# Yubo-Shankui/Bind-Your-Avatar-Implementation

Measured on AMD Instinct MI355X. Metric: denoise-steps/sec, higher is better.
Workload: dtype bf16; 1 GPU; BASELINE.json configs[1]: full transformer.forward, 49x480x720 (13x30x45 latent tokens + 226 text), 2 characters (2 ID + 2 audio), batch 1, random-init 8.6B-param architecture; layers=42, batch=1, launch=eager, parallelism=single GPU

## Files before the change

### bind_your_avatar_implementation_amd/_hip.py

```python
import ctypes
import os

from .build import LIB_PATH as _BUILT_LIB

LIB_PATH = os.environ.get("BYA_HIP_LIB") or _BUILT_LIB

_c = ctypes
_vp, _i32, _i64, _f32 = _c.c_void_p, _c.c_int32, _c.c_int64, _c.c_float


class GemmDesc(_c.Structure):
    _fields_ = [("M", _i32), ("N", _i32), ("K", _i32), ("batch", _i32),
                ("lda", _i32), ("ldw", _i32), ("ldc", _i32), ("ldres", _i32),
                ("a_batch_stride", _i64), ("c_batch_stride", _i64), ("res_batch_stride", _i64),
                ("gate_batch_stride", _i64), ("gate_split", _i32), ("act", _i32),
                ("n_split", _i32), ("c_split_stride", _i64), ("bias_rowscale", _vp), ("alpha", _f32)]


class GemmPlan(_c.Structure):
    _fields_ = [("path", _i32), ("m0", _i32), ("tail", _i32), ("split_k", _i32), ("row_chunks", _i32)]


class QkNormDesc(_c.Structure):
    _fields_ = [("qw", _vp), ("qb", _vp), ("kw", _vp), ("kb", _vp), ("cos", _vp), ("sin", _vp),
# ... 96 lines not shown
    "bya_masks_to_routing_logits": [_vp, _vp, _i32, _i32, _i32, _i32, _i32, _i32, _i32, _vp],
    "bya_vae_patches": [_vp, _vp, _vp] + [_i32] * 14 + [_vp],
    "bya_vae_groupnorm_stats": [_vp, _vp, _vp, _i64, _i32, _i32, _vp],
    "bya_vae_norm_act": [_vp, _vp, _vp, _vp, _vp, _vp, _vp, _i64, _i32, _i32, _i32, _f32, _i32, _i32, _i32, _i32, _i32, _i32,
                         _i32, _i64, _i32, _vp],
    "bya_vae_conv3d": [_vp, _vp, _vp, _vp, _vp, _i32, _i32, _i32, _i32, _i32, _i32, _i64, _i64, _i64, _vp],
    "bya_vae_upsample_pad": [_vp, _vp, _i32, _i32, _i32, _i32, _i32, _vp],
    "bya_allgather_kv": [_vp, _vp, _vp, _vp, _i64, _i64, _vp, _vp],
    "bya_alltoall_router": [_vp, _vp, _vp, _vp, _i32, _vp, _vp],
    "bya_p2p_push": [_vp, _i32, _i64, _vp, _i32, _i32, _vp, _vp],
    "bya_p2p_wait": [_vp, _i32, _vp, _i64, _vp],
    "bya_p2p_exchange": [_vp, _i32, _i64, _vp, _i32, _i32, _vp, _vp, _i64, _vp],
    "bya_p2p_poison": [_vp, _i32, _vp, _i64, _vp],
    "bya_p2p_alloc": [_i64, _i32, _c.POINTER(_vp)],
    "bya_p2p_free": [_vp],
    "bya_p2p_ipc_export": [_vp, _vp],
    "bya_p2p_ipc_import": [_vp, _c.POINTER(_vp)],
    "bya_p2p_ipc_release": [_vp],
    "bya_cfg_scheduler_step": [_vp, _i32, _i64, _vp, _vp, _vp, _vp, _vp, _i64, _c.POINTER(SchedCoef), _vp],
}

OPTIONS = {"gemm_splitk": 0, "gemm_splitk_min": 1, "gemm_tile": 2, "gemm_variant": 3, "attn_streamk": 4, "fp8_kernel": 5,
           "p2p_groups": 6, "reference_forms": 7}
REFERENCE_FORMS = {"rowgemm_chunked": 1, "kv_mix_generic": 2, "ln_generic": 4, "router_scores_wave": 8, "attn_narrow_store": 16}
ENV_OPTIONS = {
    "BYA_GEMM_SPLITK": ("gemm_splitk", int),
    "BYA_GEMM_SPLITK_MIN": ("gemm_splitk_min", int),
    "BYA_GEMM_TILE": ("gemm_tile", int),
    "BYA_GEMM_VARIANT": ("gemm_variant", lambda v: {"w8": 1, "no128": 2}.get(v, 0)),
    "BYA_ATTN_STREAMK": ("attn_streamk", int),
    "BYA_FP8_KERNEL": ("fp8_kernel", lambda v: 1 if v.startswith("1") else 0),
    "BYA_P2P_GROUPS": ("p2p_groups", int),
}

GEMM_PATHS = {0: "t128x64", 1: "t128x128", 2: "t256x128", 3: "t256x256", 4: "p256", 5: "p128", 6: "p128s", 7: "w8_256"}

ATTN_VARIANTS = {0: "d64_running_max", 1: "d64_prescaled_running_max", 2: "d64_static_bound", 3: "d128_running_max",
                 4: "d64_static_bound_w4", 5: "d64_device_bound_w4"}
KV_MIX_FORMS = {0: "mix32", 1: "one_tile"}
TINY_INSTANCES = {0: "tiny8<2>", 1: "tiny8<3>", 2: "tiny8<13>", 3: "tiny8<25>", 4: "generic<2>", 5: "generic<4>",
                  6: "generic<16>", 7: "generic<32>"}

ERRORS = {-1: "BYA_ERR_SHAPE", -2: "BYA_ERR_ALIGN", -3: "BYA_ERR_LAUNCH", -4: "BYA_ERR_UNSUPPORTED"}

_lib = None


# ... 47 lines not shown
```

### bind_your_avatar_implementation_amd/csrc/misc.hip

```cpp
#include "bya_common.h"
#include "../../include/bya.h"
#include "options.h"
#include "routing_weights.h"

namespace {

template <int MAXM>
__global__ __launch_bounds__(256) void linear_small_m_kernel(const bf16_t* __restrict__ x, const bf16_t* __restrict__ W,
                                                             const bf16_t* __restrict__ bias, bf16_t* __restrict__ out,
                                                             int M, int N, int K, int silu_in, int act_out) {
    const int lane = threadIdx.x & 63;
    const long long n = (long long)blockIdx.x * 4 + (threadIdx.x >> 6);
    if (n >= N) return;
    float acc[MAXM];
#pragma unroll
    for (int m = 0; m < MAXM; ++m) acc[m] = 0.f;
    const bf16_t* wrow = W + n * K;
    for (int k0 = lane * 8; k0 < K; k0 += 512) {
        float wv[8];
        unpack8(*reinterpret_cast<const u32x4*>(wrow + k0), wv);
#pragma unroll
        for (int m = 0; m < MAXM; ++m) {
            if (m < M) {
                float xv[8];
// ... 273 lines not shown
        v += plane(lt.i1) * lt.w1;
        if (v > 0.5f) label = id;
    }
    for (int id = 0; id < n_id; ++id) out[tok * n_id + id] = (id == label) ? (bf16_t)0x3F80 : (bf16_t)0;
}

}

extern "C" int bya_abi_version(void) { return 2; }

std::atomic<int32_t> g_bya_options[BYA_OPT_COUNT] = {
    {0},
    {0},
    {-1},
    {0},
    {1},
    {0},
    {0},
    {0},
};

extern "C" int bya_set_option(int32_t key, int32_t value) {
    static const int32_t lo[BYA_OPT_COUNT] = {0, 0, -1, 0, 0, 0, 0, 0};
    static const int32_t hi[BYA_OPT_COUNT] = {2, 1 << 20, 6, 2, 1, 1, 1024, 31};
    if (key < 0 || key >= BYA_OPT_COUNT || value < lo[key] || value > hi[key]) return BYA_ERR_SHAPE;
    if (key == BYA_OPT_P2P_GROUPS && value != 0 && value < 16) return BYA_ERR_SHAPE;
    g_bya_options[key].store(value, std::memory_order_relaxed);
    return BYA_OK;
}

extern "C" int bya_get_option(int32_t key, int32_t* value) {
    if (key < 0 || key >= BYA_OPT_COUNT || !value) return BYA_ERR_SHAPE;
    *value = g_bya_options[key].load(std::memory_order_relaxed);
    return BYA_OK;
}

extern "C" int bya_linear_small_m(const void* x, const void* W, const void* bias, void* out, int32_t M, int32_t N,
                                  int32_t K, int32_t silu_in, int32_t act_out, hipStream_t stream) {
    if (!x || !W || !out || M <= 0 || M > 8 || N <= 0 || K <= 0) return BYA_ERR_SHAPE;
    if (K % 8) return BYA_ERR_SHAPE;
    if (((uintptr_t)x | (uintptr_t)W) & 15) return BYA_ERR_ALIGN;
    if (act_out != BYA_ACT_NONE && act_out != BYA_ACT_SILU) return BYA_ERR_UNSUPPORTED;
    dim3 grid((unsigned)((N + 3) / 4));
    if (M <= 2)
        BYA_LAUNCH((linear_small_m_kernel<2>), grid, dim3(256), 0, stream, (const bf16_t*)x, (const bf16_t*)W,
                           (const bf16_t*)bias, (bf16_t*)out, M, N, K, silu_in, act_out);
    else
// ... 116 lines not shown
```

### bind_your_avatar_implementation_amd/csrc/rowgemm.hip

```cpp
#include "rowgemm_common.h"
#include "../../include/bya.h"
#include "options.h"

#ifndef BYA_ROWGEMM_ABLATE
#define BYA_ROWGEMM_ABLATE 0
#endif

namespace {

using namespace rowk;

struct RowGemmArgs {
    const bf16_t* X; const bf16_t* W; const float* colsum; const float* cvec; const bf16_t* res; bf16_t* C;
    int M, N, ldx, ldc, ldres;
    float eps;
};

constexpr int HB = 2;
constexpr int NW = CH / (4 * HB);
constexpr int SR = CH / NW;
constexpr int RB = 16 * HB * NW;
constexpr int WG_PER_CU = 1;
constexpr int AHEAD = 1;

template <bool LN, bool RES, int ACT>
__global__ __launch_bounds__(64 * NW, 2) void rowgemm512_kernel(RowGemmArgs p) {
    extern __shared__ __attribute__((aligned(16))) char smem[];
    const int tid = threadIdx.x, lane = tid & 63;
    const int wave = __builtin_amdgcn_readfirstlane(tid >> 6);

    const int nrb = (p.M + RB - 1) / RB, ncc = p.N / CH;
    const long long total = (long long)nrb * ncc;
    const int rid = (gridDim.x & 7) == 0 ? (int)((blockIdx.x & 7) * (gridDim.x >> 3) + (blockIdx.x >> 3)) : (int)blockIdx.x;
    const int q0 = (int)(total * rid / gridDim.x), q1 = (int)(total * (rid + 1) / gridDim.x);
    if (q0 >= q1) return;

    float* s_lds = reinterpret_cast<float*>(smem);
    float* c_lds = s_lds + p.N;
    char* ring = smem + p.N * 8;
    for (int i = tid; i < p.N; i += 64 * NW) {
        s_lds[i] = LN ? p.colsum[i] : 0.0f;
        c_lds[i] = p.cvec[i];
    }
    __syncthreads();

    const __amdgpu_buffer_rsrc_t rsX = __builtin_amdgcn_make_buffer_rsrc(
        (void*)p.X, 0, (int)(((long long)(p.M - 1) * p.ldx + RK) * 2), 0x00020000);
    const __amdgpu_buffer_rsrc_t rsW = __builtin_amdgcn_make_buffer_rsrc((void*)p.W, 0, p.N * RK * 2, 0x00020000);
    const __amdgpu_buffer_rsrc_t rsC = __builtin_amdgcn_make_buffer_rsrc(
        (void*)p.C, 0, (int)(((long long)(p.M - 1) * p.ldc + p.N) * 2), 0x00020000);
    const __amdgpu_buffer_rsrc_t rsR = __builtin_amdgcn_make_buffer_rsrc(
        (void*)(RES ? p.res : p.C), 0, (int)(((long long)(p.M - 1) * (RES ? p.ldres : p.ldc) + p.N) * 2), 0x00020000);
// ... 44 lines not shown
                for (int h = 0; h < HB; ++h) {
                    f32x4 sm = {0.f, 0.f, 0.f, 0.f}, gr = {0.f, 0.f, 0.f, 0.f};
#pragma unroll
                    for (int ks = 0; ks < 16; ++ks) {
                        sm = __builtin_amdgcn_mfma_f32_16x16x32_bf16(ones, xf[h][ks], sm, 0, 0, 0);
                        gr = __builtin_amdgcn_mfma_f32_16x16x32_bf16(xf[h][ks], xf[h][ks], gr, 0, 0, 0);
                    }
                    const int e = to & 3;
                    const float d = e == 0 ? gr[0] : e == 1 ? gr[1] : e == 2 ? gr[2] : gr[3];
                    const float sq = __shfl(d, (int)(to + 16 * (to >> 2)));
                    const float mu = sm[0] * (1.0f / RK);
                    const float var = fmaxf(sq * (1.0f / RK) - mu * mu, 0.0f);
                    mean[h] = mu;
                    rstd[h] = rsqrtf(var + p.eps);
                }
            }
        }
        asm volatile("s_waitcnt vmcnt(0)" ::: "memory");
#pragma unroll
        for (int h = 0; h < HB; ++h)
#pragma unroll
            for (int ks = 0; ks < 16; ++ks) asm volatile("" : "+v"(xf[h][ks]));

        for (; q < qe; ++q, ++it) {
            const int cc = q - rb * ncc, stg = it & 1;
            const uint32_t ln = lane_now(), to = ln & 15u, go = ln >> 4;
            asm volatile("s_waitcnt vmcnt(%0)" ::"i"(NJ * HB / 2) : "memory");
            __builtin_amdgcn_s_barrier();
            u32x4 rv[HB][NJ / 2];
            if (RES) {
#pragma unroll
                for (int h = 0; h < HB; ++h)
#pragma unroll
                    for (int u = 0; u < NJ / 2; ++u)
                        rv[h][u] = __builtin_bit_cast(u32x4, __builtin_amdgcn_raw_buffer_load_b128(
                            rsR, ((uint32_t)(r0 + h * 16) + to) * (uint32_t)(p.ldres * 2) +
                                     ((uint32_t)(cc * CH) + lane_col(go, u)) * 2, 0, 0));
            }
            if (q + 1 < q1) stage_chunk(q + 1, stg ^ 1);

            uint32_t wa[4];
#pragma unroll
            for (int m = 0; m < 4; ++m)
                wa[m] = ring_base + stg * STAGE_BYTES + to * 1024 + (((go ^ (to & 3)) | ((m ^ (to >> 2)) << 2)) << 4);
            f32x4 acc[HB][NJ];
#pragma unroll
            for (int h = 0; h < HB; ++h)
#pragma unroll
                for (int j = 0; j < NJ; ++j) acc[h][j] = f32x4{0.f, 0.f, 0.f, 0.f};
            bf16x8 wf[AHEAD + 1][NJ];
#pragma unroll
            for (int a = 0; a < AHEAD; ++a) read_kstep(wf[a], wa, a);
#pragma unroll
            for (int ks = 0; ks < 16; ++ks) {
                const int cur = ks % (AHEAD + 1);
                if (ks + AHEAD < 16) {
                    read_kstep(wf[(ks + AHEAD) % (AHEAD + 1)], wa, ks + AHEAD);
                    lgkm_wait<AHEAD * NJ>(wf[cur]);
                } else if (ks + 1 < 16 && AHEAD == 2) {
                    lgkm_wait<NJ>(wf[cur]);
                } else {
                    lgkm_wait<0>(wf[cur]);
                }
#pragma unroll
                for (int j = 0; j < NJ; ++j)
#pragma unroll
                    for (int h = 0; h < HB; ++h)
                        acc[h][j] = __builtin_amdgcn_mfma_f32_16x16x32_bf16(wf[cur][j], xf[h][ks], acc[h][j], 0, 0, 0);
            }

#pragma unroll
            for (int u = 0; u < NJ / 2; ++u) {
                f32x4 s0, s1, c0, c1;
                const uint32_t a = smem_base + ((uint32_t)(cc * CH) + lane_col(go, u)) * 4, ac = a + (uint32_t)p.N * 4;
                lds_read_f<0>(s0, a);
                lds_read_f<16>(s1, a);
                lds_read_f<0>(c0, ac);
                lds_read_f<16>(c1, ac);
                asm volatile("s_waitcnt lgkmcnt(0)" : "+v"(s0), "+v"(s1), "+v"(c0), "+v"(c1));
#pragma unroll
                for (int h = 0; h < HB; ++h) {
                    float v[8];
#pragma unroll
                    for (int e = 0; e < 8; ++e) {
                        const float a0 = acc[h][2 * u + (e >> 2)][e & 3];
                        const float sv = (e >> 2) ? s1[e & 3] : s0[e & 3];
                        const float cv = (e >> 2) ? c1[e & 3] : c0[e & 3];
                        float o = LN ? fmaf(rstd[h], fmaf(-mean[h], sv, a0), cv) : a0 + cv;
                        if (ACT == BYA_ACT_GELU_ERF) o = gelu_erf_f(o);
                        if (RES) o += (e & 1) ? bfhi(rv[h][u][e >> 1]) : bflo(rv[h][u][e >> 1]);
                        v[e] = o;
                    }
                    u32x4 ov;
#pragma unroll
                    for (int w2 = 0; w2 < 4; ++w2) ov[w2] = pack2bf(v[2 * w2], v[2 * w2 + 1]);
#if BYA_ROWGEMM_ABLATE & 2
                    if (ov[0] == 0x12345678u && ov[3] == 0x9abcdef0u)
#endif
                    __builtin_amdgcn_raw_buffer_store_b128(ov, rsC, ((uint32_t)(r0 + h * 16) + to) * (uint32_t)(p.ldc * 2) +
                                                                        ((uint32_t)(cc * CH) + lane_col(go, u)) * 2, 0, 0);
                }
            }
        }
    }
}

template <bool LN, bool RES, int ACT>
int launch_rowgemm(const RowGemmArgs& a, hipStream_t s) {
    const long long total = (long long)((a.M + RB - 1) / RB) * (a.N / CH);
    const int blocks = (int)(total < 256 * WG_PER_CU ? total : 256 * WG_PER_CU);
    const size_t lds = (size_t)a.N * 8 + 2 * STAGE_BYTES;
    static std::atomic<unsigned long long> attr_done{0};
    if (bya_allow_big_lds(reinterpret_cast<const void*>(rowgemm512_kernel<LN, RES, ACT>), 160 * 1024, attr_done) != BYA_OK)
        return BYA_ERR_LAUNCH;
    BYA_LAUNCH((rowgemm512_kernel<LN, RES, ACT>), dim3(blocks), dim3(64 * NW), lds, s, a);
    return hipGetLastError() == hipSuccess ? BYA_OK : BYA_ERR_LAUNCH;
}


template <bool LN, bool RES, int ACT>
__global__ __launch_bounds__(64 * NW, 2) void rowgemm512q_kernel(RowGemmArgs p) {
    static_assert(!LN, "the W-stationary form has no LayerNorm-folding instance");
    extern __shared__ __attribute__((aligned(16))) char smem[];
    const int tid = threadIdx.x, lane = tid & 63;
    const int wave = __builtin_amdgcn_readfirstlane(tid >> 6);
    const int xcd = blockIdx.x & 7, idx = blockIdx.x >> 3, per_xcd = gridDim.x >> 5;
    const int quarter = idx & 3, rgrp = xcd * per_xcd + (idx >> 2), ngroups = gridDim.x >> 2;
    const int col_base = quarter * 128;

    float* s_lds = reinterpret_cast<float*>(smem);
    float* c_lds = s_lds + 128;
    char* ring = smem + 1024;
    if (tid < 128) {
        s_lds[tid] = LN ? p.colsum[col_base + tid] : 0.0f;
        c_lds[tid] = p.cvec[col_base + tid];
    }
    const __amdgpu_buffer_rsrc_t rsX = __builtin_amdgcn_make_buffer_rsrc(
        (void*)p.X, 0, (int)(((long long)(p.M - 1) * p.ldx + RK) * 2), 0x00020000);
    const __amdgpu_buffer_rsrc_t rsW = __builtin_amdgcn_make_buffer_rsrc((void*)p.W, 0, p.N * RK * 2, 0x00020000);
// ... 185 lines not shown
#pragma unroll
        for (int j = 0; j < NJ; ++j) acc[h][j] = f32x4{0.f, 0.f, 0.f, 0.f};
    bf16x8 wf[AHEAD + 1][NJ];
#pragma unroll
    for (int a = 0; a < AHEAD; ++a) read_kstep(wf[a], wa, a);
#pragma unroll
    for (int ks = 0; ks < 16; ++ks) {
        const int cur = ks % (AHEAD + 1);
        if (ks + AHEAD < 16) {
            read_kstep(wf[(ks + AHEAD) % (AHEAD + 1)], wa, ks + AHEAD);
            lgkm_wait<AHEAD * NJ>(wf[cur]);
        } else {
            lgkm_wait<0>(wf[cur]);
        }
#pragma unroll
        for (int j = 0; j < NJ; ++j)
#pragma unroll
            for (int h = 0; h < HB; ++h)
                acc[h][j] = SWAP ? __builtin_amdgcn_mfma_f32_16x16x32_bf16(xf[h][ks], wf[cur][j], acc[h][j], 0, 0, 0)
                                 : __builtin_amdgcn_mfma_f32_16x16x32_bf16(wf[cur][j], xf[h][ks], acc[h][j], 0, 0, 0);
    }
}

template <bool WIDE>
__global__ __launch_bounds__(64 * NW, 2) void rowattn512_kernel(RowAttnArgs p) {
    extern __shared__ __attribute__((aligned(16))) char smem[];
    const int tid = threadIdx.x, lane = tid & 63;
    const int wave = __builtin_amdgcn_readfirstlane(tid >> 6);

    const long long tiles = WIDE ? 2 * p.n_groups : (p.n_groups + p.G - 1) / p.G;
    const int nrb = (int)((tiles + NW * HB - 1) / (NW * HB));
    const int total = nrb * RA_HEADS;
    const int rid = (gridDim.x & 7) == 0 ? (int)((blockIdx.x & 7) * (gridDim.x >> 3) + (blockIdx.x >> 3)) : (int)blockIdx.x;
    const int u0 = (int)((long long)total * rid / gridDim.x), u1 = (int)((long long)total * (rid + 1) / gridDim.x);
    if (u0 >= u1) return;

    float* s_lds = reinterpret_cast<float*>(smem);
    float* c_lds = s_lds + RA_N;
    float* st_lds = c_lds + RA_N + wave * (HB * 32);
    char* ring = smem + RA_CONST_BYTES;
    for (int i = tid; i < RA_N; i += 64 * NW) {
        s_lds[i] = p.colsum[i];
        c_lds[i] = p.cvec[i];
    }
    __syncthreads();

    const __amdgpu_buffer_rsrc_t rsX = __builtin_amdgcn_make_buffer_rsrc(
        (void*)p.X, 0, (int)(((long long)(p.M - 1) * p.ldx + RK) * 2), 0x00020000);
    const __amdgpu_buffer_rsrc_t rsW = __builtin_amdgcn_make_buffer_rsrc((void*)p.W, 0, RA_N * RK * 2, 0x00020000);
    const __amdgpu_buffer_rsrc_t rsO = __builtin_amdgcn_make_buffer_rsrc(
        (void*)p.O, 0, (int)(((long long)(p.M - 1) * p.ldo + RK) * 2), 0x00020000);
// ... 61 lines not shown
                for (int ks = 0; ks < 16; ++ks) {
                    sm = __builtin_amdgcn_mfma_f32_16x16x32_bf16(ones, xf[h][ks], sm, 0, 0, 0);
                    gr = __builtin_amdgcn_mfma_f32_16x16x32_bf16(xf[h][ks], xf[h][ks], gr, 0, 0, 0);
                }
                const int e = to & 3;
                const float d = e == 0 ? gr[0] : e == 1 ? gr[1] : e == 2 ? gr[2] : gr[3];
                const float sq = __shfl(d, (int)(to + 16 * (to >> 2)));
                const float mu = sm[0] * (1.0f / RK);
                const float var = fmaxf(sq * (1.0f / RK) - mu * mu, 0.0f);
                mean[h] = mu;
                rstd[h] = rsqrtf(var + p.eps);
                if (go == 0) {
                    st_lds[h * 32 + to] = mean[h];
                    st_lds[h * 32 + 16 + to] = rstd[h];
                }
            }
        }
        asm volatile("s_waitcnt vmcnt(0) lgkmcnt(0)" ::: "memory");
#pragma unroll
        for (int h = 0; h < HB; ++h)
#pragma unroll
            for (int ks = 0; ks < 16; ++ks) asm volatile("" : "+v"(xf[h][ks]));

        for (; u < ue; ++u) {
            const int head = u & (RA_HEADS - 1);
            u32x4 qf[HB][2], kf[HB][2];
            u32x2 pf[HB][WIDE ? HB : 1];
            float invl[HB];
#pragma unroll
            for (int part = 0; part < 2; ++part) {
                const uint32_t ln = lane_now(), to = ln & 15u, go = ln >> 4;
                if (part == 0) asm volatile("s_waitcnt vmcnt(%0)" ::"i"(2 * HB) : "memory");
                else asm volatile("s_waitcnt vmcnt(0)" ::: "memory");
                __builtin_amdgcn_s_barrier();
                if (3 * u + part + 1 < q_end) stage_chunk(3 * u + part + 1, stg ^ 1);
                uint32_t wa[4];
#pragma unroll
                for (int m = 0; m < 4; ++m)
                    wa[m] = ring_base + stg * STAGE_BYTES + to * 1024 + (((go ^ (to & 3)) | ((m ^ (to >> 2)) << 2)) << 4);
                f32x4 acc[HB][NJ];
                rowattn_chunk<false>(acc, xf, wa);
                const uint32_t sc_base = smem_base + (uint32_t)(part * 512 + head * 64 + LPC * go) * 4;
#pragma unroll
                for (int kb = 0; kb < 2; ++kb) {
                    f32x4 s0, s1, c0, c1;
                    const uint32_t a = sc_base + (uint32_t)(8 * kb) * 4, ac = a + (uint32_t)RA_N * 4;
                    lds_read_f<0>(s0, a);
                    lds_read_f<16>(s1, a);
                    lds_read_f<0>(c0, ac);
                    lds_read_f<16>(c1, ac);
                    asm volatile("s_waitcnt lgkmcnt(0)" : "+v"(s0), "+v"(s1), "+v"(c0), "+v"(c1));
#pragma unroll
                    for (int h = 0; h < HB; ++h) {
                        float v[8];
#pragma unroll
                        for (int e = 0; e < 8; ++e) {
                            const float a0 = acc[h][2 * kb + (e >> 2)][e & 3];
                            const float sv = (e >> 2) ? s1[e & 3] : s0[e & 3];
                            const float cv = (e >> 2) ? c1[e & 3] : c0[e & 3];
                            v[e] = fmaf(rstd[h], fmaf(-mean[h], sv, a0), cv);
                        }
                        u32x4 w;
#pragma unroll
                        for (int w2 = 0; w2 < 4; ++w2) w[w2] = pack2bf(v[2 * w2], v[2 * w2 + 1]);
                        if (part == 0) qf[h][kb] = w; else kf[h][kb] = w;
                    }
                }
                stg ^= 1;
            }
            constexpr int NKT = WIDE ? HB : 1;
#pragma unroll
            for (int h = 0; h < HB; ++h) {
                float sv[NKT][4];
                float mx = -INFINITY;
#pragma unroll
                for (int hk = 0; hk < NKT; ++hk) {
                    const int kt = WIDE ? hk : h;
                    f32x4 st = {0.f, 0.f, 0.f, 0.f};
#pragma unroll
                    for (int kb = 0; kb < 2; ++kb)
                        st = __builtin_amdgcn_mfma_f32_16x16x32_bf16(__builtin_bit_cast(bf16x8, kf[kt][kb]),
                                                                     __builtin_bit_cast(bf16x8, qf[h][kb]), st, 0, 0, 0);
#pragma unroll
                    for (int e = 0; e < 4; ++e) {
                        sv[hk][e] = (kmask >> (4 * hk + e)) & 1u ? st[e] : -INFINITY;
                        mx = fmaxf(mx, sv[hk][e]);
                    }
                }
                mx = fmaxf(mx, __shfl_xor(mx, 16));
                mx = fmaxf(mx, __shfl_xor(mx, 32));
                float l = 0.f;
#pragma unroll
                for (int hk = 0; hk < NKT; ++hk) {
                    float pe[4];
#pragma unroll
                    for (int e = 0; e < 4; ++e) {
                        pe[e] = __builtin_amdgcn_exp2f((sv[hk][e] - mx) * p.scale_log2);
                        l += pe[e];
                    }
                    pf[h][hk][0] = pack2bf(pe[0], pe[1]);
                    pf[h][hk][1] = pack2bf(pe[2], pe[3]);
                }
                l += __shfl_xor(l, 16);
                l += __shfl_xor(l, 32);
                invl[h] = __builtin_amdgcn_rcpf(l);
            }
            {
                const uint32_t ln = lane_now(), to = ln & 15u, go = ln >> 4;
                asm volatile("s_waitcnt vmcnt(0)" ::: "memory");
                __builtin_amdgcn_s_barrier();
                if (3 * u + 3 < q_end) stage_chunk(3 * u + 3, stg ^ 1);
                uint32_t wa[4];
#pragma unroll
                for (int m = 0; m < 4; ++m)
                    wa[m] = ring_base + stg * STAGE_BYTES + to * 1024 + (((go ^ (to & 3)) | ((m ^ (to >> 2)) << 2)) << 4);
                f32x4 acc[HB][NJ];
                rowattn_chunk<true>(acc, xf, wa);
                const uint32_t col = (uint32_t)(1024 + head * 64) + LPC * (to >> 2) + (to & 3);
                float sj[NJ], cj[NJ];
#pragma unroll
                for (int j = 0; j < NJ; ++j) {
                    sj[j] = s_lds[col + 4 * j];
                    cj[j] = c_lds[col + 4 * j];
                }
                auto make_vt = [&](int h, u32x2 (&vt)[NJ]) {
                    f32x4 m4, r4;
                    lds_read_f<0>(m4, st_base + (uint32_t)(h * 32 + 4 * go) * 4);
                    lds_read_f<64>(r4, st_base + (uint32_t)(h * 32 + 4 * go) * 4);
                    asm volatile("s_waitcnt lgkmcnt(0)" : "+v"(m4), "+v"(r4));
#pragma unroll
                    for (int j = 0; j < NJ; ++j) {
                        float vv[4];
#pragma unroll
                        for (int e = 0; e < 4; ++e) vv[e] = fmaf(r4[e], fmaf(-m4[e], sj[j], acc[h][j][e]), cj[j]);
                        vt[j][0] = pack2bf(vv[0], vv[1]);
                        vt[j][1] = pack2bf(vv[2], vv[3]);
                    }
                };
                u32x2 vt[WIDE ? HB : 1][NJ];
                if constexpr (WIDE) {
#pragma unroll
                    for (int h = 0; h < HB; ++h) make_vt(h, vt[h]);
                }
#pragma unroll
                for (int h = 0; h < HB; ++h) {
                    if constexpr (!WIDE) make_vt(h, vt[0]);
                    float ov[16];
#pragma unroll
                    for (int j = 0; j < NJ; ++j) {
                        f32x4 o = {0.f, 0.f, 0.f, 0.f};
#pragma unroll
                        for (int hk = 0; hk < NKT; ++hk)
                            o = __builtin_amdgcn_mfma_f32_16x16x16bf16_1k(__builtin_bit_cast(s16x4, vt[WIDE ? hk : 0][j]),
                                                                          __builtin_bit_cast(s16x4, pf[h][hk]), o, 0, 0, 0);
#pragma unroll
                        for (int e = 0; e < 4; ++e) ov[4 * j + e] = o[e] * invl[h];
                    }
                    const uint32_t off = rowi[h] * (uint32_t)(p.ldo * 2) + ((uint32_t)(head * 64) + LPC * go) * 2;
                    __builtin_amdgcn_raw_buffer_store_b128(pack8(ov), rsO, off, 0, 0);
                    __builtin_amdgcn_raw_buffer_store_b128(pack8(ov + 8), rsO, off + 16, 0, 0);
                }
                stg ^= 1;
            }
        }
    }
}

}

extern "C" int bya_rowgemm512(const void* X, const void* W, const float* colsum, const float* cvec, const void* res,
                              void* C, int32_t M, int32_t N, int32_t ldx, int32_t ldc, int32_t ldres, int32_t ln,
                              float eps, int32_t act, int32_t nsplit, hipStream_t stream) {
    (void)nsplit;
    if (!X || !W || !cvec || !C || M <= 0 || N <= 0) return BYA_ERR_SHAPE;
    if (ln && !colsum) return BYA_ERR_SHAPE;
    if (N % CH != 0 || N > 4096) return BYA_ERR_SHAPE;
    if (ldx < RK || ldc < N || (res && ldres < N) || ldx % 8 || ldc % 8 || (res && ldres % 8)) return BYA_ERR_ALIGN;
    if (((uintptr_t)X | (uintptr_t)W | (uintptr_t)C | (uintptr_t)res) & 15) return BYA_ERR_ALIGN;
    if ((long long)M * ldx * 2 >= (1LL << 31) || (long long)M * ldc * 2 >= (1LL << 31)) return BYA_ERR_SHAPE;
    if (act != BYA_ACT_NONE && act != BYA_ACT_GELU_ERF) return BYA_ERR_UNSUPPORTED;
    RowGemmArgs a;
    a.X = (const bf16_t*)X; a.W = (const bf16_t*)W; a.colsum = colsum; a.cvec = cvec; a.res = (const bf16_t*)res;
    a.C = (bf16_t*)C; a.M = M; a.N = N; a.ldx = ldx; a.ldc = ldc; a.ldres = res ? ldres : ldc;
    a.eps = eps;
    const bool gelu = act == BYA_ACT_GELU_ERF;
    if (N == 512 && !ln && M >= 2048 && M <= 65536 && !bya_ref_form(BYA_REF_ROWGEMM_CHUNKED)) {
        if (res) return gelu ? launch_rowgemm_q<false, true, BYA_ACT_GELU_ERF>(a, stream) : launch_rowgemm_q<false, true, BYA_ACT_NONE>(a, stream);
// ... 13 lines not shown

extern "C" int bya_router_group_attn(const void* X, const void* Wqkv, const float* colsum, const float* cvec, void* O,
                                     int32_t M, int32_t ldx, int32_t ldo, int32_t L, int64_t n_outer, int64_t n_inner,
                                     int64_t outer_stride, int64_t seq_stride, float eps, float scale, hipStream_t stream) {
    if (!X || !Wqkv || !colsum || !cvec || !O || M <= 0 || n_outer <= 0 || n_inner <= 0) return BYA_ERR_SHAPE;
    if (L < 1 || L > 32) return BYA_ERR_UNSUPPORTED;
    if (outer_stride < 0 || seq_stride < 0) return BYA_ERR_SHAPE;
    if ((n_outer - 1) * outer_stride + (n_inner - 1) + (int64_t)(L - 1) * seq_stride >= M) return BYA_ERR_SHAPE;
    if (ldx < RK || ldo < RK || ldx % 8 || ldo % 8) return BYA_ERR_ALIGN;
    if (((uintptr_t)X | (uintptr_t)Wqkv | (uintptr_t)O) & 15) return BYA_ERR_ALIGN;
    if (((long long)M + 1) * ldx * 2 >= (1LL << 31) || ((long long)M + 1) * ldo * 2 >= (1LL << 31)) return BYA_ERR_SHAPE;
    RowAttnArgs a;
    a.X = (const bf16_t*)X; a.W = (const bf16_t*)Wqkv; a.colsum = colsum; a.cvec = cvec; a.O = (bf16_t*)O;
    a.M = M; a.ldx = ldx; a.ldo = ldo; a.L = L;
    const bool wide = L > 16;
    a.P = L <= 1 ? 1 : L <= 2 ? 2 : L <= 4 ? 4 : L <= 8 ? 8 : 16;
    a.G = 16 / a.P;
    a.n_groups = n_outer * n_inner; a.n_inner = n_inner; a.outer_stride = outer_stride; a.seq_stride = seq_stride;
    a.eps = eps; a.scale_log2 = scale * 1.4426950408889634f;
    const long long tiles = wide ? 2 * a.n_groups : (a.n_groups + a.G - 1) / a.G;
    const long long total = ((tiles + NW * HB - 1) / (NW * HB)) * RA_HEADS;
    const int blocks = (int)(total < 256 ? total : 256);
    const size_t lds = (size_t)RA_CONST_BYTES + 2 * STAGE_BYTES;
    static std::atomic<unsigned long long> attr_done{0};
    static std::atomic<unsigned long long> attr_done_w{0};
    if (wide) {
        if (bya_allow_big_lds(reinterpret_cast<const void*>(rowattn512_kernel<true>), 160 * 1024, attr_done_w) != BYA_OK) return BYA_ERR_LAUNCH;
        BYA_LAUNCH(rowattn512_kernel<true>, dim3(blocks), dim3(64 * NW), lds, stream, a);
    } else {
        if (bya_allow_big_lds(reinterpret_cast<const void*>(rowattn512_kernel<false>), 160 * 1024, attr_done) != BYA_OK) return BYA_ERR_LAUNCH;
        BYA_LAUNCH(rowattn512_kernel<false>, dim3(blocks), dim3(64 * NW), lds, stream, a);
    }
    return hipGetLastError() == hipSuccess ? BYA_OK : BYA_ERR_LAUNCH;
}
```

### include/bya.h

```cpp
#ifndef BYA_H
#define BYA_H

#include <stdint.h>

#ifdef __cplusplus
extern "C" {
#endif
#if defined(__GNUC__) || defined(__clang__)
#pragma GCC visibility push(default)
#endif

#ifndef __HIP_PLATFORM_AMD__
typedef struct ihipStream_t* hipStream_t;
#endif

enum { BYA_ACT_NONE = 0, BYA_ACT_GELU_TANH = 1, BYA_ACT_GELU_ERF = 2, BYA_ACT_RELU = 3, BYA_ACT_SILU = 4,
       BYA_ACT_LEAKY_RELU = 5,
       BYA_ACT_GELU_TANH_IEEE = 6  };

int bya_abi_version(void);

enum bya_option {
    BYA_OPT_GEMM_SPLITK = 0,
    BYA_OPT_GEMM_SPLITK_MIN = 1,
    BYA_OPT_GEMM_TILE = 2,
    BYA_OPT_GEMM_VARIANT = 3,
    BYA_OPT_ATTN_STREAMK = 4,
    BYA_OPT_FP8_KERNEL = 5,
    BYA_OPT_P2P_GROUPS = 6,
    BYA_OPT_REFERENCE_FORMS = 7,
    BYA_OPT_COUNT = 8
};
enum { BYA_REF_ROWGEMM_CHUNKED = 1,
       BYA_REF_KV_MIX_GENERIC = 2,
       BYA_REF_LN_GENERIC = 4,
       BYA_REF_ROUTER_SCORES_WAVE = 8,
       BYA_REF_ATTN_NARROW_STORE = 16   };
int bya_set_option(int32_t key, int32_t value);
int bya_get_option(int32_t key, int32_t* value);

#define BYA_CALIBRATION_OPERAND_BYTES (256LL * 256 * 16 * 16)
#define BYA_CALIBRATION_FLOP_PER_ITER (256.0 * 4 * 2.0 * 128 * 128 * 32)
int bya_mfma_calibration(const void* operands, int64_t operand_bytes, void* sink, int32_t iters, hipStream_t stream);

typedef struct bya_gemm_desc {
    int32_t M, N, K;
    int32_t batch;
    int32_t lda, ldw, ldc, ldres;
    int64_t a_batch_stride, c_batch_stride, res_batch_stride, gate_batch_stride;
    int32_t gate_split;
    int32_t act;
    int32_t n_split;
    int64_t c_split_stride;
    const float* bias_rowscale;
    float alpha;
} bya_gemm_desc;

int bya_gemm_bf16(const void* A, const void* W, const void* bias, void* C, const void* res,
                  const void* gate0, const void* gate1, const bya_gemm_desc* desc, hipStream_t stream);

// ... 283 lines not shown
```

Baseline: 2.898 steps/s.

## Stagger late waves' epilogues behind next chunk in rowattn and rowgemm kernels

Splits the waves of each workgroup so the upper half defers its epilogue (LN-correction, softmax, V-projection/store) to run after the next chunk's barrier and staging. Early and late waves then interleave MFMA and VALU/LDS phases instead of all hitting the same phase in lockstep. For rowattn the staggered form becomes the default; for rowgemm it sits behind a new reference-form flag and stays off. The cost is more live registers (acc, qf/kf kept across iterations), extra template instantiations, and subtler wait-count logic.

```diff
diff --git a/bind_your_avatar_implementation_amd/_hip.py b/bind_your_avatar_implementation_amd/_hip.py
--- a/bind_your_avatar_implementation_amd/_hip.py
+++ b/bind_your_avatar_implementation_amd/_hip.py
@@ -142,7 +142,8 @@
 
 OPTIONS = {"gemm_splitk": 0, "gemm_splitk_min": 1, "gemm_tile": 2, "gemm_variant": 3, "attn_streamk": 4, "fp8_kernel": 5,
            "p2p_groups": 6, "reference_forms": 7}
-REFERENCE_FORMS = {"rowgemm_chunked": 1, "kv_mix_generic": 2, "ln_generic": 4, "router_scores_wave": 8, "attn_narrow_store": 16}
+REFERENCE_FORMS = {"rowgemm_chunked": 1, "kv_mix_generic": 2, "ln_generic": 4, "router_scores_wave": 8, "attn_narrow_store": 16,
+                   "rowattn_lockstep": 32, "rowgemm_staggered": 64}
 ENV_OPTIONS = {
     "BYA_GEMM_SPLITK": ("gemm_splitk", int),
     "BYA_GEMM_SPLITK_MIN": ("gemm_splitk_min", int),
diff --git a/bind_your_avatar_implementation_amd/csrc/misc.hip b/bind_your_avatar_implementation_amd/csrc/misc.hip
--- a/bind_your_avatar_implementation_amd/csrc/misc.hip
+++ b/bind_your_avatar_implementation_amd/csrc/misc.hip
@@ -319,7 +319,7 @@
 
 extern "C" int bya_set_option(int32_t key, int32_t value) {
     static const int32_t lo[BYA_OPT_COUNT] = {0, 0, -1, 0, 0, 0, 0, 0};
-    static const int32_t hi[BYA_OPT_COUNT] = {2, 1 << 20, 6, 2, 1, 1, 1024, 31};
+    static const int32_t hi[BYA_OPT_COUNT] = {2, 1 << 20, 6, 2, 1, 1, 1024, 127};
     if (key < 0 || key >= BYA_OPT_COUNT || value < lo[key] || value > hi[key]) return BYA_ERR_SHAPE;
     if (key == BYA_OPT_P2P_GROUPS && value != 0 && value < 16) return BYA_ERR_SHAPE;
     g_bya_options[key].store(value, std::memory_order_relaxed);
diff --git a/bind_your_avatar_implementation_amd/csrc/rowgemm.hip b/bind_your_avatar_implementation_amd/csrc/rowgemm.hip
--- a/bind_your_avatar_implementation_amd/csrc/rowgemm.hip
+++ b/bind_your_avatar_implementation_amd/csrc/rowgemm.hip
@@ -23,11 +23,12 @@
 constexpr int WG_PER_CU = 1;
 constexpr int AHEAD = 1;
 
-template <bool LN, bool RES, int ACT>
+template <bool LN, bool RES, int ACT, bool STAG>
 __global__ __launch_bounds__(64 * NW, 2) void rowgemm512_kernel(RowGemmArgs p) {
     extern __shared__ __attribute__((aligned(16))) char smem[];
     const int tid = threadIdx.x, lane = tid & 63;
     const int wave = __builtin_amdgcn_readfirstlane(tid >> 6);
+    const bool late = STAG && wave >= NW / 2;
 
     const int nrb = (p.M + RB - 1) / RB, ncc = p.N / CH;
     const long long total = (long long)nrb * ncc;
@@ -118,53 +119,20 @@
 #pragma unroll
             for (int ks = 0; ks < 16; ++ks) asm volatile("" : "+v"(xf[h][ks]));
 
-        for (; q < qe; ++q, ++it) {
-            const int cc = q - rb * ncc, stg = it & 1;
+        f32x4 acc[HB][NJ];
+        u32x4 rv[HB][NJ / 2];
+        auto load_residual = [&](int cc) {
             const uint32_t ln = lane_now(), to = ln & 15u, go = ln >> 4;
-            asm volatile("s_waitcnt vmcnt(%0)" ::"i"(NJ * HB / 2) : "memory");
-            __builtin_amdgcn_s_barrier();
-            u32x4 rv[HB][NJ / 2];
-            if (RES) {
-#pragma unroll
-                for (int h = 0; h < HB; ++h)
-#pragma unroll
-                    for (int u = 0; u < NJ / 2; ++u)
-                        rv[h][u] = __builtin_bit_cast(u32x4, __builtin_amdgcn_raw_buffer_load_b128(
-                            rsR, ((uint32_t)(r0 + h * 16) + to) * (uint32_t)(p.ldres * 2) +
-                                     ((uint32_t)(cc * CH) + lane_col(go, u)) * 2, 0, 0));
-            }
-            if (q + 1 < q1) stage_chunk(q + 1, stg ^ 1);
-
-            uint32_t wa[4];
-#pragma unroll
-            for (int m = 0; m < 4; ++m)
-                wa[m] = ring_base + stg * STAGE_BYTES + to * 1024 + (((go ^ (to & 3)) | ((m ^ (to >> 2)) << 2)) << 4);
-            f32x4 acc[HB][NJ];
 #pragma unroll
             for (int h = 0; h < HB; ++h)
 #pragma unroll
-                for (int j = 0; j < NJ; ++j) acc[h][j] = f32x4{0.f, 0.f, 0.f, 0.f};
-            bf16x8 wf[AHEAD + 1][NJ];
-#pragma unroll
-            for (int a = 0; a < AHEAD; ++a) read_kstep(wf[a], wa, a);
-#pragma unroll
-            for (int ks = 0; ks < 16; ++ks) {
-                const int cur = ks % (AHEAD + 1);
-                if (ks + AHEAD < 16) {
-                    read_kstep(wf[(ks + AHEAD) % (AHEAD + 1)], wa, ks + AHEAD);
-                    lgkm_wait<AHEAD * NJ>(wf[cur]);
-                } else if (ks + 1 < 16 && AHEAD == 2) {
-                    lgkm_wait<NJ>(wf[cur]);
-                } else {
-                    lgkm_wait<0>(wf[cur]);
-                }
-#pragma unroll
-                for (int j = 0; j < NJ; ++j)
-#pragma unroll
-                    for (int h = 0; h < HB; ++h)
-                        acc[h][j] = __builtin_amdgcn_mfma_f32_16x16x32_bf16(wf[cur][j], xf[h][ks], acc[h][j], 0, 0, 0);
-            }
-
+                for (int u = 0; u < NJ / 2; ++u)
+                    rv[h][u] = __builtin_bit_cast(u32x4, __builtin_amdgcn_raw_buffer_load_b128(
+                        rsR, ((uint32_t)(r0 + h * 16) + to) * (uint32_t)(p.ldres * 2) +
+                                 ((uint32_t)(cc * CH) + lane_col(go, u)) * 2, 0, 0));
+        };
+        auto epilogue = [&](int cc) {
+            const uint32_t ln = lane_now(), to = ln & 15u, go = ln >> 4;
 #pragma unroll
             for (int u = 0; u < NJ / 2; ++u) {
                 f32x4 s0, s1, c0, c1;
@@ -197,20 +165,73 @@
                                                                         ((uint32_t)(cc * CH) + lane_col(go, u)) * 2, 0, 0);
                 }
             }
-        }
-    }
-}
-
-template <bool LN, bool RES, int ACT>
-int launch_rowgemm(const RowGemmArgs& a, hipStream_t s) {
+        };
+
+        const int qs = q;
+        for (; q < qe; ++q, ++it) {
+            const int cc = q - rb * ncc, stg = it & 1;
+            const uint32_t ln = lane_now(), to = ln & 15u, go = ln >> 4;
+            if (STAG && late && !RES && q <= qs + 1) asm volatile("s_waitcnt vmcnt(0)" ::: "memory");
+            else asm volatile("s_waitcnt vmcnt(%0)" ::"i"(NJ * HB / 2) : "memory");
+            __builtin_amdgcn_s_barrier();
+            if (RES && !late) load_residual(cc);
+            if (q + 1 < q1) stage_chunk(q + 1, stg ^ 1);
+            if (STAG && late) {
+                if (q > qs) epilogue(cc - 1);
+                if (RES) load_residual(cc);
+            }
+
+            uint32_t wa[4];
+#pragma unroll
+            for (int m = 0; m < 4; ++m)
+                wa[m] = ring_base + stg * STAGE_BYTES + to * 1024 + (((go ^ (to & 3)) | ((m ^ (to >> 2)) << 2)) << 4);
+#pragma unroll
+            for (int h = 0; h < HB; ++h)
+#pragma unroll
+                for (int j = 0; j < NJ; ++j) acc[h][j] = f32x4{0.f, 0.f, 0.f, 0.f};
+            bf16x8 wf[AHEAD + 1][NJ];
+#pragma unroll
+            for (int a = 0; a < AHEAD; ++a) read_kstep(wf[a], wa, a);
+#pragma unroll
+            for (int ks = 0; ks < 16; ++ks) {
+                const int cur = ks % (AHEAD + 1);
+                if (ks + AHEAD < 16) {
+                    read_kstep(wf[(ks + AHEAD) % (AHEAD + 1)], wa, ks + AHEAD);
+                    lgkm_wait<AHEAD * NJ>(wf[cur]);
+                } else if (ks + 1 < 16 && AHEAD == 2) {
+                    lgkm_wait<NJ>(wf[cur]);
+                } else {
+                    lgkm_wait<0>(wf[cur]);
+                }
+#pragma unroll
+                for (int j = 0; j < NJ; ++j)
+#pragma unroll
+                    for (int h = 0; h < HB; ++h)
+                        acc[h][j] = __builtin_amdgcn_mfma_f32_16x16x32_bf16(wf[cur][j], xf[h][ks], acc[h][j], 0, 0, 0);
+            }
+
+            if (!(STAG && late)) epilogue(cc);
+        }
+        if (STAG && late) epilogue(qe - 1 - rb * ncc);
+    }
+}
+
+template <bool LN, bool RES, int ACT, bool STAG>
+int launch_rowgemm_form(const RowGemmArgs& a, hipStream_t s) {
     const long long total = (long long)((a.M + RB - 1) / RB) * (a.N / CH);
     const int blocks = (int)(total < 256 * WG_PER_CU ? total : 256 * WG_PER_CU);
     const size_t lds = (size_t)a.N * 8 + 2 * STAGE_BYTES;
     static std::atomic<unsigned long long> attr_done{0};
-    if (bya_allow_big_lds(reinterpret_cast<const void*>(rowgemm512_kernel<LN, RES, ACT>), 160 * 1024, attr_done) != BYA_OK)
+    if (bya_allow_big_lds(reinterpret_cast<const void*>(rowgemm512_kernel<LN, RES, ACT, STAG>), 160 * 1024, attr_done) != BYA_OK)
         return BYA_ERR_LAUNCH;
-    BYA_LAUNCH((rowgemm512_kernel<LN, RES, ACT>), dim3(blocks), dim3(64 * NW), lds, s, a);
+    BYA_LAUNCH((rowgemm512_kernel<LN, RES, ACT, STAG>), dim3(blocks), dim3(64 * NW), lds, s, a);
     return hipGetLastError() == hipSuccess ? BYA_OK : BYA_ERR_LAUNCH;
+}
+
+template <bool LN, bool RES, int ACT>
+int launch_rowgemm(const RowGemmArgs& a, hipStream_t s) {
+    if (bya_ref_form(BYA_REF_ROWGEMM_STAGGERED)) return launch_rowgemm_form<LN, RES, ACT, true>(a, s);
+    return launch_rowgemm_form<LN, RES, ACT, false>(a, s);
 }
 
 
@@ -442,11 +463,12 @@
     }
 }
 
-template <bool WIDE>
+template <bool WIDE, bool STAG>
 __global__ __launch_bounds__(64 * NW, 2) void rowattn512_kernel(RowAttnArgs p) {
     extern __shared__ __attribute__((aligned(16))) char smem[];
     const int tid = threadIdx.x, lane = tid & 63;
     const int wave = __builtin_amdgcn_readfirstlane(tid >> 6);
+    const bool late = STAG && wave >= NW / 2;
 
     const long long tiles = WIDE ? 2 * p.n_groups : (p.n_groups + p.G - 1) / p.G;
     const int nrb = (int)((tiles + NW * HB - 1) / (NW * HB));
@@ -554,53 +576,47 @@
 #pragma unroll
             for (int ks = 0; ks < 16; ++ks) asm volatile("" : "+v"(xf[h][ks]));
 
-        for (; u < ue; ++u) {
-            const int head = u & (RA_HEADS - 1);
-            u32x4 qf[HB][2], kf[HB][2];
-            u32x2 pf[HB][WIDE ? HB : 1];
-            float invl[HB];
-#pragma unroll
-            for (int part = 0; part < 2; ++part) {
-                const uint32_t ln = lane_now(), to = ln & 15u, go = ln >> 4;
-                if (part == 0) asm volatile("s_waitcnt vmcnt(%0)" ::"i"(2 * HB) : "memory");
-                else asm volatile("s_waitcnt vmcnt(0)" ::: "memory");
-                __builtin_amdgcn_s_barrier();
-                if (3 * u + part + 1 < q_end) stage_chunk(3 * u + part + 1, stg ^ 1);
-                uint32_t wa[4];
-#pragma unroll
-                for (int m = 0; m < 4; ++m)
-                    wa[m] = ring_base + stg * STAGE_BYTES + to * 1024 + (((go ^ (to & 3)) | ((m ^ (to >> 2)) << 2)) << 4);
-                f32x4 acc[HB][NJ];
-                rowattn_chunk<false>(acc, xf, wa);
-                const uint32_t sc_base = smem_base + (uint32_t)(part * 512 + head * 64 + LPC * go) * 4;
-#pragma unroll
-                for (int kb = 0; kb < 2; ++kb) {
-                    f32x4 s0, s1, c0, c1;
-                    const uint32_t a = sc_base + (uint32_t)(8 * kb) * 4, ac = a + (uint32_t)RA_N * 4;
-                    lds_read_f<0>(s0, a);
-                    lds_read_f<16>(s1, a);
-                    lds_read_f<0>(c0, ac);
-                    lds_read_f<16>(c1, ac);
-                    asm volatile("s_waitcnt lgkmcnt(0)" : "+v"(s0), "+v"(s1), "+v"(c0), "+v"(c1));
-#pragma unroll
-                    for (int h = 0; h < HB; ++h) {
-                        float v[8];
-#pragma unroll
-                        for (int e = 0; e < 8; ++e) {
-                            const float a0 = acc[h][2 * kb + (e >> 2)][e & 3];
-                            const float sv = (e >> 2) ? s1[e & 3] : s0[e & 3];
-                            const float cv = (e >> 2) ? c1[e & 3] : c0[e & 3];
-                            v[e] = fmaf(rstd[h], fmaf(-mean[h], sv, a0), cv);
-                        }
-                        u32x4 w;
-#pragma unroll
-                        for (int w2 = 0; w2 < 4; ++w2) w[w2] = pack2bf(v[2 * w2], v[2 * w2 + 1]);
-                        if (part == 0) qf[h][kb] = w; else kf[h][kb] = w;
+        constexpr int NKT = WIDE ? HB : 1;
+        f32x4 acc[HB][NJ];
+        u32x4 qf[HB][2], kf[HB][2];
+        u32x2 pf[HB][NKT];
+        float invl[HB];
+        auto chunk_addr = [&](uint32_t (&wa)[4]) {
+            const uint32_t ln = lane_now(), to = ln & 15u, go = ln >> 4;
+#pragma unroll
+            for (int m = 0; m < 4; ++m)
+                wa[m] = ring_base + stg * STAGE_BYTES + to * 1024 + (((go ^ (to & 3)) | ((m ^ (to >> 2)) << 2)) << 4);
+        };
+        auto epi_qk = [&](int part, int head, u32x4 (&dst)[HB][2]) {
+            const uint32_t ln = lane_now(), go = ln >> 4;
+            const uint32_t sc_base = smem_base + (uint32_t)(part * 512 + head * 64 + LPC * go) * 4;
+#pragma unroll
+            for (int kb = 0; kb < 2; ++kb) {
+                f32x4 s0, s1, c0, c1;
+                const uint32_t a = sc_base + (uint32_t)(8 * kb) * 4, ac = a + (uint32_t)RA_N * 4;
+                lds_read_f<0>(s0, a);
+                lds_read_f<16>(s1, a);
+                lds_read_f<0>(c0, ac);
+                lds_read_f<16>(c1, ac);
+                asm volatile("s_waitcnt lgkmcnt(0)" : "+v"(s0), "+v"(s1), "+v"(c0), "+v"(c1));
+#pragma unroll
+                for (int h = 0; h < HB; ++h) {
+                    float v[8];
+#pragma unroll
+                    for (int e = 0; e < 8; ++e) {
+                        const float a0 = acc[h][2 * kb + (e >> 2)][e & 3];
+                        const float sv = (e >> 2) ? s1[e & 3] : s0[e & 3];
+                        const float cv = (e >> 2) ? c1[e & 3] : c0[e & 3];
+                        v[e] = fmaf(rstd[h], fmaf(-mean[h], sv, a0), cv);
                     }
-                }
-                stg ^= 1;
-            }
-            constexpr int NKT = WIDE ? HB : 1;
+                    u32x4 w;
+#pragma unroll
+                    for (int w2 = 0; w2 < 4; ++w2) w[w2] = pack2bf(v[2 * w2], v[2 * w2 + 1]);
+                    dst[h][kb] = w;
+                }
+            }
+        };
+        auto softmax = [&]() {
 #pragma unroll
             for (int h = 0; h < HB; ++h) {
                 float sv[NKT][4];
@@ -637,64 +653,91 @@
                 l += __shfl_xor(l, 32);
                 invl[h] = __builtin_amdgcn_rcpf(l);
             }
+        };
+        auto finish_v = [&](int head) {
+            const uint32_t ln = lane_now(), to = ln & 15u, go = ln >> 4;
+            const uint32_t col = (uint32_t)(1024 + head * 64) + LPC * (to >> 2) + (to & 3);
+            float sj[NJ], cj[NJ];
+#pragma unroll
+            for (int j = 0; j < NJ; ++j) {
+                sj[j] = s_lds[col + 4 * j];
+                cj[j] = c_lds[col + 4 * j];
+            }
+            auto make_vt = [&](int h, u32x2 (&vt)[NJ]) {
+                f32x4 m4, r4;
+                lds_read_f<0>(m4, st_base + (uint32_t)(h * 32 + 4 * go) * 4);
+                lds_read_f<64>(r4, st_base + (uint32_t)(h * 32 + 4 * go) * 4);
+                asm volatile("s_waitcnt lgkmcnt(0)" : "+v"(m4), "+v"(r4));
+#pragma unroll
+                for (int j = 0; j < NJ; ++j) {
+                    float vv[4];
+#pragma unroll
+                    for (int e = 0; e < 4; ++e) vv[e] = fmaf(r4[e], fmaf(-m4[e], sj[j], acc[h][j][e]), cj[j]);
+                    vt[j][0] = pack2bf(vv[0], vv[1]);
+                    vt[j][1] = pack2bf(vv[2], vv[3]);
+                }
+            };
+            u32x2 vt[WIDE ? HB : 1][NJ];
+            if constexpr (WIDE) {
+#pragma unroll
+                for (int h = 0; h < HB; ++h) make_vt(h, vt[h]);
+            }
+#pragma unroll
+            for (int h = 0; h < HB; ++h) {
+                if constexpr (!WIDE) make_vt(h, vt[0]);
+                float ov[16];
+#pragma unroll
+                for (int j = 0; j < NJ; ++j) {
+                    f32x4 o = {0.f, 0.f, 0.f, 0.f};
+#pragma unroll
+                    for (int hk = 0; hk < NKT; ++hk)
+                        o = __builtin_amdgcn_mfma_f32_16x16x16bf16_1k(__builtin_bit_cast(s16x4, vt[WIDE ? hk : 0][j]),
+                                                                      __builtin_bit_cast(s16x4, pf[h][hk]), o, 0, 0, 0);
+#pragma unroll
+                    for (int e = 0; e < 4; ++e) ov[4 * j + e] = o[e] * invl[h];
+                }
+                const uint32_t off = rowi[h] * (uint32_t)(p.ldo * 2) + ((uint32_t)(head * 64) + LPC * go) * 2;
+                __builtin_amdgcn_raw_buffer_store_b128(pack8(ov), rsO, off, 0, 0);
+                __builtin_amdgcn_raw_buffer_store_b128(pack8(ov + 8), rsO, off + 16, 0, 0);
+            }
+        };
+
+        const int us = u;
+        for (; u < ue; ++u) {
+            const int head = u & (RA_HEADS - 1);
+#pragma unroll
+            for (int part = 0; part < 2; ++part) {
+                if (late ? (part == 1 && u > us) : part == 0) asm volatile("s_waitcnt vmcnt(%0)" ::"i"(2 * HB) : "memory");
+                else asm volatile("s_waitcnt vmcnt(0)" ::: "memory");
+                __builtin_amdgcn_s_barrier();
+                if (3 * u + part + 1 < q_end) stage_chunk(3 * u + part + 1, stg ^ 1);
+                if (STAG && late) {
+                    if (part == 0) { if (u > us) finish_v((u - 1) & (RA_HEADS - 1)); }
+                    else epi_qk(0, head, qf);
+                }
+                uint32_t wa[4];
+                chunk_addr(wa);
+                rowattn_chunk<false>(acc, xf, wa);
+                if (!(STAG && late)) { if (part == 0) epi_qk(0, head, qf); else epi_qk(1, head, kf); }
+                stg ^= 1;
+            }
+            if (!(STAG && late)) softmax();
             {
-                const uint32_t ln = lane_now(), to = ln & 15u, go = ln >> 4;
                 asm volatile("s_waitcnt vmcnt(0)" ::: "memory");
                 __builtin_amdgcn_s_barrier();
                 if (3 * u + 3 < q_end) stage_chunk(3 * u + 3, stg ^ 1);
+                if (STAG && late) {
+                    epi_qk(1, head, kf);
+                    softmax();
+                }
                 uint32_t wa[4];
-#pragma unroll
-                for (int m = 0; m < 4; ++m)
-                    wa[m] = ring_base + stg * STAGE_BYTES + to * 1024 + (((go ^ (to & 3)) | ((m ^ (to >> 2)) << 2)) << 4);
-                f32x4 acc[HB][NJ];
+                chunk_addr(wa);
                 rowattn_chunk<true>(acc, xf, wa);
-                const uint32_t col = (uint32_t)(1024 + head * 64) + LPC * (to >> 2) + (to & 3);
-                float sj[NJ], cj[NJ];
-#pragma unroll
-                for (int j = 0; j < NJ; ++j) {
-                    sj[j] = s_lds[col + 4 * j];
-                    cj[j] = c_lds[col + 4 * j];
-                }
-                auto make_vt = [&](int h, u32x2 (&vt)[NJ]) {
-                    f32x4 m4, r4;
-                    lds_read_f<0>(m4, st_base + (uint32_t)(h * 32 + 4 * go) * 4);
-                    lds_read_f<64>(r4, st_base + (uint32_t)(h * 32 + 4 * go) * 4);
-                    asm volatile("s_waitcnt lgkmcnt(0)" : "+v"(m4), "+v"(r4));
-#pragma unroll
-                    for (int j = 0; j < NJ; ++j) {
-                        float vv[4];
-#pragma unroll
-                        for (int e = 0; e < 4; ++e) vv[e] = fmaf(r4[e], fmaf(-m4[e], sj[j], acc[h][j][e]), cj[j]);
-                        vt[j][0] = pack2bf(vv[0], vv[1]);
-                        vt[j][1] = pack2bf(vv[2], vv[3]);
-                    }
-                };
-                u32x2 vt[WIDE ? HB : 1][NJ];
-                if constexpr (WIDE) {
-#pragma unroll
-                    for (int h = 0; h < HB; ++h) make_vt(h, vt[h]);
-                }
-#pragma unroll
-                for (int h = 0; h < HB; ++h) {
-                    if constexpr (!WIDE) make_vt(h, vt[0]);
-                    float ov[16];
-#pragma unroll
-                    for (int j = 0; j < NJ; ++j) {
-                        f32x4 o = {0.f, 0.f, 0.f, 0.f};
-#pragma unroll
-                        for (int hk = 0; hk < NKT; ++hk)
-                            o = __builtin_amdgcn_mfma_f32_16x16x16bf16_1k(__builtin_bit_cast(s16x4, vt[WIDE ? hk : 0][j]),
-                                                                          __builtin_bit_cast(s16x4, pf[h][hk]), o, 0, 0, 0);
-#pragma unroll
-                        for (int e = 0; e < 4; ++e) ov[4 * j + e] = o[e] * invl[h];
-                    }
-                    const uint32_t off = rowi[h] * (uint32_t)(p.ldo * 2) + ((uint32_t)(head * 64) + LPC * go) * 2;
-                    __builtin_amdgcn_raw_buffer_store_b128(pack8(ov), rsO, off, 0, 0);
-                    __builtin_amdgcn_raw_buffer_store_b128(pack8(ov + 8), rsO, off + 16, 0, 0);
-                }
+                if (!(STAG && late)) finish_v(head);
                 stg ^= 1;
             }
         }
+        if (STAG && late) finish_v((ue - 1) & (RA_HEADS - 1));
     }
 }
 
@@ -754,14 +797,15 @@
     const long long total = ((tiles + NW * HB - 1) / (NW * HB)) * RA_HEADS;
     const int blocks = (int)(total < 256 ? total : 256);
     const size_t lds = (size_t)RA_CONST_BYTES + 2 * STAGE_BYTES;
-    static std::atomic<unsigned long long> attr_done{0};
-    static std::atomic<unsigned long long> attr_done_w{0};
-    if (wide) {
-        if (bya_allow_big_lds(reinterpret_cast<const void*>(rowattn512_kernel<true>), 160 * 1024, attr_done_w) != BYA_OK) return BYA_ERR_LAUNCH;
-        BYA_LAUNCH(rowattn512_kernel<true>, dim3(blocks), dim3(64 * NW), lds, stream, a);
-    } else {
-        if (bya_allow_big_lds(reinterpret_cast<const void*>(rowattn512_kernel<false>), 160 * 1024, attr_done) != BYA_OK) return BYA_ERR_LAUNCH;
-        BYA_LAUNCH(rowattn512_kernel<false>, dim3(blocks), dim3(64 * NW), lds, stream, a);
-    }
+    const bool stag = !bya_ref_form(BYA_REF_ROWATTN_LOCKSTEP);
+    auto launch = [&](auto kernel, std::atomic<unsigned long long>& attr_done) -> int {
+        if (bya_allow_big_lds(reinterpret_cast<const void*>(kernel), 160 * 1024, attr_done) != BYA_OK) return BYA_ERR_LAUNCH;
+        BYA_LAUNCH(kernel, dim3(blocks), dim3(64 * NW), lds, stream, a);
+        return BYA_OK;
+    };
+    static std::atomic<unsigned long long> attr_done[4] = {{0}, {0}, {0}, {0}};
+    const int rc = wide ? (stag ? launch(rowattn512_kernel<true, true>, attr_done[3]) : launch(rowattn512_kernel<true, false>, attr_done[2]))
+                        : (stag ? launch(rowattn512_kernel<false, true>, attr_done[1]) : launch(rowattn512_kernel<false, false>, attr_done[0]));
+    if (rc != BYA_OK) return rc;
     return hipGetLastError() == hipSuccess ? BYA_OK : BYA_ERR_LAUNCH;
 }
diff --git a/include/bya.h b/include/bya.h
--- a/include/bya.h
+++ b/include/bya.h
@@ -35,7 +35,9 @@
        BYA_REF_KV_MIX_GENERIC = 2,
        BYA_REF_LN_GENERIC = 4,
        BYA_REF_ROUTER_SCORES_WAVE = 8,
-       BYA_REF_ATTN_NARROW_STORE = 16   };
+       BYA_REF_ATTN_NARROW_STORE = 16,
+       BYA_REF_ROWATTN_LOCKSTEP = 32,
+       BYA_REF_ROWGEMM_STAGGERED = 64   };
 int bya_set_option(int32_t key, int32_t value);
 int bya_get_option(int32_t key, int32_t* value);
 
```

Result: no change. 2.903 steps/s (median of 6 runs) (+0.2%).
